# mims-harvard/ProCyon

Measured on AMD Instinct MI355X. Metric: phenotype-gen tokens/sec (ProCyon-Full greedy generation, end to end), higher is better.
Workload: dtype bf16; 1 GPU; configs[1]: ProCyon-Full (ESM2-650M + Llama-3-8B geometry=full) bf16 batch=1, 1024-residue protein, 512-token prompt, 256-token greedy generation; parallelism=single GPU

## Files before the change

### procyon_amd/_lib.py

```python
from __future__ import annotations

import ctypes as C
import os

_HERE = os.path.dirname(os.path.abspath(__file__))
LIB_PATH = os.environ.get("PCY_LIB") or os.path.join(_HERE, "libpcy.so")

EPI_STORE, EPI_RESID, EPI_GELU_ERF, EPI_GELU_ESM, EPI_SWIGLU = range(5)
POOL_MEAN, POOL_MEAN_CORRECTED, POOL_MAX = range(3)
ABI_VERSION = 10
(DISPATCH_GEMM_128, DISPATCH_GEMM_64, DISPATCH_GEMM_BIG, DISPATCH_GEMM_BIG_PERSIST, DISPATCH_GEMM_SPLITK, DISPATCH_GEMM_FP8, DISPATCH_ATTN_FAST,
 DISPATCH_DEC_STEP_GQA, DISPATCH_GEMM_MID, DISPATCH_ESM_GRAPH, DISPATCH_DEC_STEP_MHA, DISPATCH_DEC_LAYER, DISPATCH_DEC_STEP_NB, DISPATCH_DEC_STEP_MB,
 DISPATCH_DEC_LOOP_STREAM, DISPATCH_DEC_LOOP_MFMA) = range(16)
DISPATCH_DECODE = dict(step_gqa=DISPATCH_DEC_STEP_GQA, step_mha=DISPATCH_DEC_STEP_MHA, layer=DISPATCH_DEC_LAYER, step_nb=DISPATCH_DEC_STEP_NB,
                       step_mb=DISPATCH_DEC_STEP_MB, loop_stream=DISPATCH_DEC_LOOP_STREAM, loop_mfma=DISPATCH_DEC_LOOP_MFMA)

vp = C.c_void_p
i32 = C.c_int32
ci = C.c_int


class MlpDesc(C.Structure):
    _fields_ = [("n_layers", i32), ("dims", i32 * 9), ("w", vp * 8), ("b", vp * 8)]


class EsmLayer(C.Structure):
    _fields_ = [(n, vp) for n in ("wqkv", "bqkv", "wo", "bo", "ln1_w", "ln1_b", "w1", "b1", "w2", "b2", "ln2_w", "ln2_b")]


class EsmDesc(C.Structure):
    _fields_ = [("d", i32), ("n_layers", i32), ("n_heads", i32), ("ffn", i32), ("vocab", i32), ("ln_eps", C.c_float),
                ("rope_mode", i32), ("embed", vp), ("final_ln_w", vp), ("final_ln_b", vp), ("rope_cos", vp),
                ("rope_sin", vp), ("layers", C.POINTER(EsmLayer))]


class LlamaLayer(C.Structure):
# ... 118 lines not shown
```

### procyon_amd/csrc/pcy_elem.hip

```cpp
#include "pcy_internal.h"

namespace {

constexpr int NT = 256;

__global__ __launch_bounds__(NT) void rmsnorm_kernel(const bf16_t* __restrict__ x, const bf16_t* __restrict__ w,
                                                     bf16_t* __restrict__ y, int d, float eps, int cast) {
  __shared__ float red[NT / 64];
  const bf16_t* xr = x + (size_t)blockIdx.x * d;
  bf16_t* yr = y + (size_t)blockIdx.x * d;
  float ss = 0.f;
  for (int k = threadIdx.x * 8; k < d; k += NT * 8) {
    const uint4 v = *reinterpret_cast<const uint4*>(xr + k);
    const uint32_t u[4] = {v.x, v.y, v.z, v.w};
#pragma unroll
    for (int j = 0; j < 4; ++j) { float a = lo_bf(u[j]), b = hi_bf(u[j]); ss += a * a + b * b; }
  }
  ss = block_sum<NT>(ss, red);
  const float rstd = rsqrtf(ss / (float)d + eps);
  for (int k = threadIdx.x * 8; k < d; k += NT * 8) {
    const uint4 v = *reinterpret_cast<const uint4*>(xr + k);
    const uint4 g = *reinterpret_cast<const uint4*>(w + k);
    const uint32_t u[4] = {v.x, v.y, v.z, v.w}, gg[4] = {g.x, g.y, g.z, g.w};
    uint32_t o[4];
// ... 334 lines not shown
      wsum[((size_t)p * POOL_CH + ch) * d + c + e] = a;
      wcnt[((size_t)p * POOL_CH + ch) * d + c + e] = n;
    }
  }
}
__global__ __launch_bounds__(NT) void pool_finish_kernel(const float* __restrict__ wsum, const int* __restrict__ wcnt, int d, int mode,
                                                         bf16_t* __restrict__ out) {
  const int p = blockIdx.x, c = blockIdx.y * NT + threadIdx.x;
  if (c >= d) return;
  float a = wsum[(size_t)p * POOL_CH * d + c];
  int n = wcnt[(size_t)p * POOL_CH * d + c];
  for (int ch = 1; ch < POOL_CH; ++ch) {
    const float v = wsum[((size_t)p * POOL_CH + ch) * d + c];
    if (mode == 2) a = fmaxf(a, v);
    else { a += v; n += wcnt[((size_t)p * POOL_CH + ch) * d + c]; }
  }
  out[(size_t)p * d + c] = (mode == 2) ? f2bf(a) : f2bf(rbf(a) / (float)n);
}

constexpr int PICK_NT = 256;
constexpr int PICK_NB = 64;
struct PickPartial { float mx; int idx; float se; int pad; };

__global__ __launch_bounds__(PICK_NT) void pick_stage1_kernel(const bf16_t* __restrict__ logits, int V, PickPartial* __restrict__ part) {
  __shared__ float redv[PICK_NT / 64];
  __shared__ int redi[PICK_NT / 64];
  __shared__ float red[PICK_NT / 64];
  const int b = blockIdx.y, c = blockIdx.x;
  const int chunk = (V + PICK_NB - 1) / PICK_NB;
  const int lo = c * chunk, hi = (lo + chunk) < V ? (lo + chunk) : V;
  const bf16_t* lg = logits + (size_t)b * V;
  float best = -INFINITY;
  int bi = 0x7fffffff;
  for (int i = lo + threadIdx.x; i < hi; i += PICK_NT) {
    const float v = bf2f(lg[i]);
    if (v > best || (v == best && i < bi)) { best = v; bi = i; }
  }
#pragma unroll
  for (int o = 32; o > 0; o >>= 1) {
    const float ov = __shfl_xor(best, o, 64);
    const int oi = __shfl_xor(bi, o, 64);
    if (ov > best || (ov == best && oi < bi)) { best = ov; bi = oi; }
  }
  const int w = threadIdx.x >> 6;
  if ((threadIdx.x & 63) == 0) { redv[w] = best; redi[w] = bi; }
  __syncthreads();
  best = redv[0]; bi = redi[0];
  for (int i = 1; i < PICK_NT / 64; ++i)
    if (redv[i] > best || (redv[i] == best && redi[i] < bi)) { best = redv[i]; bi = redi[i]; }
  float se = 0.f;
  for (int i = lo + threadIdx.x; i < hi; i += PICK_NT) se += expf(bf2f(lg[i]) - best);
  se = block_sum<PICK_NT>(se, red);
  if (threadIdx.x == 0) part[b * PICK_NB + c] = PickPartial{best, bi, (lo < hi) ? se : 0.f, 0};
}

__global__ __launch_bounds__(256) void pick_stage2_kernel(const bf16_t* __restrict__ logits, int V, const PickPartial* __restrict__ part,
                                                          int32_t* __restrict__ next_tok, int32_t* __restrict__ tokens_out, int max_steps,
                                                          float* __restrict__ logprob, int32_t* __restrict__ step_dev, int32_t* __restrict__ pos_dev,
                                                          int advance_pos, int B) {
  const int l = threadIdx.x & 63;
  const int step = *step_dev;
  for (int b = threadIdx.x >> 6; b < B; b += 4) {
    const PickPartial pp = part[b * PICK_NB + l];
    float best = pp.mx;
    int bi = pp.idx;
#pragma unroll
    for (int o = 32; o > 0; o >>= 1) {
      const float ov = __shfl_xor(best, o, 64);
      const int oi = __shfl_xor(bi, o, 64);
      if (ov > best || (ov == best && oi < bi)) { best = ov; bi = oi; }
    }
    float se = pp.se * expf(pp.mx - best);
    se = wave_sum(se);
    if (l == 0) {
      const float lsm = rbf((bf2f(logits[(size_t)b * V + bi]) - best) - logf(se));
      logprob[b] += lsm;
      next_tok[b] = bi;
      tokens_out[(size_t)b * max_steps + step] = bi;
    }
  }
  __syncthreads();
  if (threadIdx.x == 0) { if (advance_pos) *pos_dev += 1; *step_dev = step + 1; }
}

constexpr int SMP_NT = 1024;

__global__ __launch_bounds__(PICK_NT) void sample_stage1_kernel(const bf16_t* __restrict__ logits, int V, float temperature,
                                                                float4* __restrict__ part) {
  __shared__ float red[PICK_NT / 64];
  const int b = blockIdx.y, c = blockIdx.x;
  const int chunk = (V + PICK_NB - 1) / PICK_NB;
  const int lo = c * chunk, hi = (lo + chunk) < V ? (lo + chunk) : V;
  const bf16_t* lg = logits + (size_t)b * V;
  const bool scaled = temperature != 1.0f;
  float mr = -INFINITY, ms = -INFINITY;
  for (int i = lo + threadIdx.x; i < hi; i += PICK_NT) {
    const float v = bf2f(lg[i]);
    mr = fmaxf(mr, v);
    ms = fmaxf(ms, scaled ? rbf(v / temperature) : v);
  }
  mr = block_max<PICK_NT>(mr, red);
  ms = block_max<PICK_NT>(ms, red);
  float sr = 0.f, ss = 0.f;
  for (int i = lo + threadIdx.x; i < hi; i += PICK_NT) {
    const float v = bf2f(lg[i]);
// ... 832 lines not shown
    for (int q = 0; q < nseq; ++q) { out[q] = acc; acc += (cu[q + 1] - cu[q] + pad - 1) / pad * pad; }
    out[nseq] = acc;
  }
}
void pcy_launch_vt_offsets(hipStream_t s, const int32_t* cu, int nseq, int pad, int32_t* vt_cu_out) {
  hipLaunchKernelGGL(vt_offsets_kernel, dim3(1), dim3(64), 0, s, cu, nseq, pad, vt_cu_out);
}
void pcy_launch_transpose_v(hipStream_t s, const bf16_t* buf, int ld, int vcol0, int nh, int dh, const int32_t* cu,
                            const int32_t* vt_cu, int nseq, int max_len, bf16_t* vt, int vt_total) {
  if (nseq <= 0) return;
  const int maxpad = (max_len + 63) / 64 * 64;
  hipLaunchKernelGGL(transpose_v_kernel, dim3((maxpad + 63) / 64, nh * dh / 64, nseq), dim3(NT), 0, s, buf, ld, vcol0, dh, cu, vt_cu, vt, vt_total);
}
size_t pcy_pool_ws_bytes(int nprot, int d) { return (size_t)nprot * POOL_CH * d * 8; }
void pcy_launch_pool(hipStream_t s, const bf16_t* h, int d, const int32_t* seg, const int32_t* rng, int nprot, int mode, bf16_t* out,
                     void* ws) {
  if (nprot <= 0) return;
  float* wsum = reinterpret_cast<float*>(ws);
  int* wcnt = reinterpret_cast<int*>(wsum + (size_t)nprot * POOL_CH * d);
  hipLaunchKernelGGL(pool_partial_kernel, dim3(nprot, (d + 511) / 512, POOL_CH), dim3(NT), 0, s, h, d, seg, rng, mode, wsum, wcnt);
  hipLaunchKernelGGL(pool_finish_kernel, dim3(nprot, (d + NT - 1) / NT), dim3(NT), 0, s, wsum, wcnt, d, mode, out);
}
void pcy_launch_greedy_pick(hipStream_t s, const bf16_t* logits, int B, int V, int32_t* next_tok, int32_t* tokens_out,
                            int max_steps, float* logprob, int32_t* pos_dev, int32_t* step_dev, int advance_pos, void* partials) {
  hipLaunchKernelGGL(pick_stage1_kernel, dim3(PICK_NB, B), dim3(PICK_NT), 0, s, logits, V, reinterpret_cast<PickPartial*>(partials));
  hipLaunchKernelGGL(pick_stage2_kernel, dim3(1), dim3(256), 0, s, logits, V, reinterpret_cast<const PickPartial*>(partials), next_tok,
                     tokens_out, max_steps, logprob, step_dev, pos_dev, advance_pos, B);
}
int pcy_sample_max_vocab() { return SMP_NT * SMP_KMAX; }
void pcy_launch_sample_step(hipStream_t s, const bf16_t* logits, int B, int V, float temperature, float nucleus_p, const float* uniforms,
                            unsigned* hist, bf16_t* probs_out, int32_t* next_tok, int32_t* tokens_out, int max_steps, float* logprob,
                            int32_t* pos_dev, int32_t* step_dev, int advance_pos, void* partials, bf16_t* pbits) {
  hipLaunchKernelGGL(sample_stage1_kernel, dim3(PICK_NB, B), dim3(PICK_NT), 0, s, logits, V, temperature, reinterpret_cast<float4*>(partials));
  hipLaunchKernelGGL(sample_probs_kernel, dim3(PICK_NB, B), dim3(PICK_NT), 0, s, logits, V, reinterpret_cast<const float4*>(partials), temperature,
                     nucleus_p > 0.f ? 1 : 0, hist, pbits);
  hipLaunchKernelGGL(sample_stage2_kernel, dim3(B), dim3(SMP_NT), 0, s, logits, V, reinterpret_cast<const float4*>(partials), temperature,
                     nucleus_p, uniforms, hist, probs_out, next_tok, tokens_out, max_steps, logprob, step_dev, B, pbits);
  hipLaunchKernelGGL(sample_advance_kernel, dim3(1), dim3(64), 0, s, pos_dev, step_dev, advance_pos);
}
void pcy_launch_copy_rows(hipStream_t s, const bf16_t* src, int lds_, bf16_t* dst, int ldd, const int32_t* rows, int nrows, int d) {
  if (nrows > 0) hipLaunchKernelGGL(copy_rows_kernel, dim3(nrows), dim3(NT), 0, s, src, lds_, dst, ldd, rows, d);
}
void pcy_launch_l2norm_rows(hipStream_t s, const bf16_t* x, bf16_t* y, int rows, int d, float eps) {
  if (rows > 0) hipLaunchKernelGGL(l2norm_rows_kernel, dim3(rows), dim3(NT), 0, s, x, y, d, eps);
}
void pcy_launch_retrieval_rank(hipStream_t s, const bf16_t* sims, int Q, int N, int k, int32_t* idx_out, bf16_t* score_out) {
  if (Q > 0 && N > 0 && k > 0)
// ... 34 lines not shown
```

### procyon_amd/csrc/pcy_engine.hip

```cpp
#include <stdio.h>
#include <stdlib.h>
#include <stdarg.h>
#include <string.h>
#include <dlfcn.h>
#include <vector>

#include "../../include/pcy.h"
#include "pcy_internal.h"

namespace {

thread_local char g_err[512] = "";

int fail(int code, const char* fmt, ...) {
  va_list ap;
  va_start(ap, fmt);
  vsnprintf(g_err, sizeof(g_err), fmt, ap);
  va_end(ap);
  return code;
}

#define HIP_TRY(expr)                                                                       \
  do {                                                                                      \
    hipError_t e_ = (expr);                                                                 \
// ... 1 lines not shown
  } while (0)

inline size_t align_up(size_t v, size_t a) { return (v + a - 1) / a * a; }

}

void pcy_set_error(const char* fmt, ...) {
  va_list ap;
  va_start(ap, fmt);
  vsnprintf(g_err, sizeof(g_err), fmt, ap);
  va_end(ap);
}

struct DecodeGraphKey {
  int kind;
  int B;
  PcySwitches sw;
  const void *model, *layers, *embed, *kv_k, *kv_v, *pos, *step, *next_tok, *logits, *keep;
  int Tmax, kv_B;
  const void *ws, *mc_tags, *mb_flags, *nb_tags, *dev_layers;
  uint64_t layers_fp;
  const void *tokens_out, *logprob, *logits_all;
  int logits_all_ld, max_steps;
  pcy_beam_state beam_state;
  const void *logits_rec, *beam_ws;
  int beam, group_size, kv_t0;
  uint32_t penalty_bits;
};

struct pcy_ctx {
  int device = 0;
  hipStream_t stream = nullptr;
  hipStream_t cap_stream = nullptr;
  char* ws = nullptr;
  size_t ws_bytes = 0;
  hipEvent_t ev0 = nullptr, ev1 = nullptr;
  hipGraphExec_t graph = nullptr;
  DecodeGraphKey graph_key = {};
  int n_cu = 0;
  unsigned* xwg_err = nullptr;
  unsigned* ao_sync = nullptr;
  uint32_t* mc_tags = nullptr;
  const void* mc_tags_model = nullptr;
  size_t mc_tags_words = 0;
  PcySwitches mc_tags_sw = {};
  uint64_t layers_fp = 0;
  PcyLayerWeightsDev* dev_layers = nullptr;
  uint32_t* nb_tags[9] = {};
  unsigned* nb_sync = nullptr;
  unsigned* mb_flags = nullptr;
  size_t mb_flags_words = 0;
  unsigned* mb_sync = nullptr;
  uint32_t* op_tags = nullptr;
  size_t op_tags_words = 0;
  unsigned* smp_hist = nullptr;
  int smp_hist_rows = 0;
  bf16_t* smp_pbits = nullptr;
  size_t smp_pbits_elems = 0;
  char* beam_ws = nullptr;
  size_t beam_ws_bytes = 0;

  struct GraphSlot { uint64_t key[16]; hipGraphExec_t exec; unsigned long long stamp; };
  static constexpr int N_GSLOTS = 8;
  GraphSlot gslots[N_GSLOTS] = {};
  unsigned long long gstamp = 0;
  void drop_gslots() {
    for (auto& g : gslots) {
      if (g.exec) hipGraphExecDestroy(g.exec);
      g = GraphSlot{};
    }
  }

  int reserve(size_t bytes) {
    static const bool poison = [] { const char* e = getenv("PCY_DEBUG_POISON_WS"); return e && atoi(e) != 0; }();
    if (poison && ws && bytes <= ws_bytes) HIP_TRY(hipMemsetAsync(ws, 0xFF, ws_bytes, stream));
    if (bytes <= ws_bytes) return 0;
    if (ws) {
      HIP_TRY(hipStreamSynchronize(stream));
      HIP_TRY(hipFree(ws));
      ws = nullptr; ws_bytes = 0;
    }
    drop_graph();
// ... 66 lines not shown
}
bool decode_mb_covers(const pcy_ctx* c, const pcy_llama_desc* m, int B, const PcySwitches& sw) {
  return B >= 9 && B <= 32 && B <= sw.mb_max && m->d == 4096 && m->ffn == 14336 && m->n_heads == 32 && m->n_kv_heads == 8 && m->head_dim == 128 && c->n_cu >= 256;
}
size_t tag_words_per_layer(const pcy_llama_desc* m) {
  return (size_t)m->ffn + (size_t)m->d + (size_t)(m->n_heads + 2 * m->n_kv_heads) * m->head_dim + (size_t)m->n_heads * m->head_dim;
}

int ensure_sync_words(pcy_ctx* c) {
  if (!c->n_cu) {
    hipDeviceProp_t prop;
    HIP_TRY(hipGetDeviceProperties(&prop, c->device));
    c->n_cu = prop.multiProcessorCount;
  }
  if (!c->xwg_err) {
    HIP_TRY(hipHostMalloc(reinterpret_cast<void**>(&c->xwg_err), 64, hipHostMallocMapped | hipHostMallocCoherent));
    memset(c->xwg_err, 0, 64);
  }
  if (!c->ao_sync) {
    const size_t bytes = (size_t)(64 + 2 * AO_MAX_LAYERS * AO_FLAGS) * sizeof(unsigned);
    HIP_TRY(hipMalloc(reinterpret_cast<void**>(&c->ao_sync), bytes));
    HIP_TRY(hipMemset(c->ao_sync, 0, bytes));
  }
  return 0;
}
uint64_t layers_fingerprint(const pcy_llama_desc* m) {
  uint64_t h = 1469598103934665603ull;
  auto mix = [&](const void* p) { h = (h ^ (uint64_t)(uintptr_t)p) * 1099511628211ull; };
  mix(m->layers);
  for (int l = 0; l < m->n_layers; ++l) {
    const pcy_llama_layer& L = m->layers[l];
    mix(L.ln1); mix(L.wqkv); mix(L.wo); mix(L.ln2); mix(L.wgu); mix(L.wdown);
  }
  return h;
}
int ensure_decode_state(pcy_ctx* c, const pcy_llama_desc* m, int B, const PcySwitches& sw) {
  if (int r = ensure_sync_words(c)) return r;
  const size_t words = (size_t)m->n_layers * (tag_words_per_layer(m) + 32 * 256);
  const uint64_t fp = layers_fingerprint(m);
  if (c->mc_tags_model != m || c->mc_tags_words != words || c->mc_tags_sw != sw || c->layers_fp != fp) {
    HIP_TRY(hipStreamSynchronize(c->stream));
    c->drop_graph();
    if (c->mc_tags) HIP_TRY(hipFree(c->mc_tags));
    c->mc_tags = nullptr;
    HIP_TRY(hipMalloc(reinterpret_cast<void**>(&c->mc_tags), words * 4));
    HIP_TRY(hipMemset(c->mc_tags, 0, words * 4));
// ... 156 lines not shown
  PcyDecodeStepArgs sa{};
  sa.layers = cx.c->dev_layers; sa.n_layers = cx.m->n_layers; sa.kv_layer_stride = cx.layer_stride;
  sa.tags = tags; sa.tag_stride = tag_stride; sa.xflags_stride = xflags_stride;
  sa.x_lines = tags + (size_t)cx.m->n_layers * tag_stride; sa.x_lines_stride = line_stride;
  return sa;
}
PcyGemvArgs proj_args(const DecodeCx& cx, const DecodePlan& p, const void* W, const void* ln, const bf16_t* in, int K, bf16_t* out, int N, int epi,
                      bool splitk, int krot, int* xn_ready) {
  const pcy_llama_desc* m = cx.m;
  PcyGemvArgs g{};
  g.W = (const bf16_t*)W; g.x = in; g.y = out; g.N = N; g.K = K; g.B = cx.B; g.ldx = K; g.ldy = N; g.epi = epi;
  g.force_stream = p.nb_on; g.krot = krot;
  if (splitk) { g.splitk_ws = cx.sk_ws; g.splitk_ws_bytes = cx.sk_bytes; }
  if (epi == EPI_RESID) {
    g.resid = out;
    if (p.batched && cx.B <= 32) { g.next_rms_w = (const bf16_t*)ln; g.next_xn = cx.xn; g.fused_next = xn_ready; g.rms_eps = m->rms_eps; g.rms_cast = m->rms_cast; }
  } else {
    g.rms_eps = m->rms_eps; g.rms_cast = m->rms_cast;
    if (p.batched) g.x = cx.xn; else g.rms_w = (const bf16_t*)ln;
  }
  return g;
}

void enqueue_decode(pcy_ctx* c, const pcy_llama_desc* m, const pcy_kv_cache* kv, const pcy_gen_state* st, int B, const PcySwitches& sw, bool layers_only = false) {
  hipStream_t s = c->stream;
  const int d = m->d, H = m->n_heads, dh = m->head_dim, F = m->ffn;
  const DecodeCx cx = decode_cx(c, m, kv, st, B);
  const DecodePlan p = plan_decode(c, m, kv, B, sw);
  if (layers_only) {
    if (p.epoch_word) pcy_launch_bump(s, p.epoch_word);
    if (p.tag_word) pcy_launch_bump(s, p.tag_word);
  } else {
    pcy_launch_embed_tokens_dev(s, (const bf16_t*)m->embed, st->next_tok, cx.x, B, d, p.epoch_word, p.tag_word);
  }
  const size_t tag_stride = tag_words_per_layer(m);
  bool step_done = false;
  bool try_layer = p.path == DEC_STEP_GQA || p.path == DEC_STEP_MHA || p.path == DEC_LAYERS;
  int xn_ready = 0;
  if (p.path == DEC_STEP_NB) {
    const PcyDecodeStepArgs sa = step_args(cx, c->nb_tags[B], pcy_decode_nb_tag_words(B), 2 * AO_FLAGS, pcy_decode_nb_line_words(B));
    step_done = pcy_launch_decode_step_nb(s, c->device, attn_args(cx, p, -1), block_args(cx, p.tag_word, mc_trace(sw)), mlp_args(cx, p.tag_word), sa, c->n_cu,
                                          c->ao_sync, B, sw.nb_ub);
    if (step_done) ++g_pcy_dispatch[PCY_DISPATCH_DEC_STEP_NB];
  } else if (p.path == DEC_STEP_GQA || p.path == DEC_STEP_MHA) {
    const PcyDecodeStepArgs sa = step_args(cx, c->mc_tags, tag_stride, AO_FLAGS, 32 * 256);
    step_done = pcy_launch_decode_step(s, attn_args(cx, p, -1), block_args(cx, p.tag_word, mc_trace(sw)), mlp_args(cx, p.tag_word), sa, c->n_cu,
                                       c->ao_sync);
  } else if (p.path == DEC_STEP_MB) {
    PcyMbArgs ma{};
    ma.layers = c->dev_layers; ma.n_layers = m->n_layers; ma.final_norm = (const bf16_t*)m->final_norm;
    ma.x = cx.x; ma.xn = cx.xn; ma.ao = cx.ao; ma.act = cx.act;
    ma.qkv_ws = cx.sk_ws; ma.sk_ws = cx.sk_ws + (size_t)2 * B * cx.qkvw;
    ma.kcache = (bf16_t*)kv->k; ma.vcache = (bf16_t*)kv->v; ma.kv_layer_stride = cx.layer_stride; ma.Bcache = kv->B;
    ma.pos_dev = st->pos; ma.cos_t = (const bf16_t*)m->rope_cos; ma.sin_t = (const bf16_t*)m->rope_sin; ma.keep = st->keep; ma.ld_keep = kv->Tmax;
    ma.B = B; ma.Tmax = kv->Tmax; ma.scale = 1.0f / sqrtf((float)dh); ma.rms_eps = m->rms_eps; ma.rms_cast = m->rms_cast;
// ... 48 lines not shown
}

__global__ void store_logits_kernel(const bf16_t* __restrict__ logits, bf16_t* __restrict__ all, const int32_t* step_dev,
                                    int B, int V, int ld) {
  const size_t step = (size_t)(*step_dev);
  const int chunks = (V + 7) / 8;
  const bool vec = (ld % 8 == 0) && ((reinterpret_cast<uintptr_t>(all) & 15) == 0);
  for (size_t i = (size_t)blockIdx.x * blockDim.x + threadIdx.x; i < (size_t)B * chunks; i += (size_t)gridDim.x * blockDim.x) {
    const int b = (int)(i / chunks), c = (int)(i % chunks);
    const bf16_t* src = logits + (size_t)b * V + c * 8;
    bf16_t* dst = all + (step * B + b) * ld + c * 8;
    if (vec && c * 8 + 8 <= V) {
      const uint32_t w0 = src[0] | ((uint32_t)src[1] << 16), w1 = src[2] | ((uint32_t)src[3] << 16);
      const uint32_t w2 = src[4] | ((uint32_t)src[5] << 16), w3 = src[6] | ((uint32_t)src[7] << 16);
      *reinterpret_cast<uint4*>(dst) = make_uint4(w0, w1, w2, w3);
    } else {
      for (int e = 0; e < 8 && c * 8 + e < V; ++e) dst[e] = src[e];
    }
  }
}
void enqueue_store_logits(hipStream_t s, const void* logits, void* all, int ld, const int32_t* step_dev, int B, int V) {
  if (all) hipLaunchKernelGGL(store_logits_kernel, dim3(B >= 8 ? 256 : 64), dim3(256), 0, s, (const bf16_t*)logits, (bf16_t*)all, step_dev, B, V, ld > 0 ? ld : V);
}
void enqueue_pick(pcy_ctx* c, const pcy_llama_desc* m, const pcy_gen_state* st, int B, int advance_pos, int Tmax) {
  enqueue_store_logits(c->stream, st->logits, st->logits_all, st->logits_all_ld, st->step, B, m->vocab);
  pcy_launch_greedy_pick(c->stream, (const bf16_t*)st->logits, B, m->vocab, st->next_tok, st->tokens_out, st->max_steps,
                         st->logprob, st->pos, st->step, advance_pos, carve_decode_ws(c->ws, m, B, Tmax).partials);
}

void enqueue_sample(pcy_ctx* c, const pcy_llama_desc* m, const pcy_gen_state* st, int B, int advance_pos, int Tmax, float temperature,
                    float nucleus_p, const float* uniforms, bf16_t* probs_out) {
  hipStream_t s = c->stream;
  if (nucleus_p > 0.f) temperature = 1.0f;
  enqueue_store_logits(s, st->logits, st->logits_all, st->logits_all_ld, st->step, B, m->vocab);
  void* partials = carve_decode_ws(c->ws, m, B, Tmax).partials;
  pcy_launch_sample_step(s, (const bf16_t*)st->logits, B, m->vocab, temperature, nucleus_p, uniforms, c->smp_hist, probs_out, st->next_tok,
                         st->tokens_out, st->max_steps, st->logprob, st->pos, st->step, advance_pos, partials, c->smp_pbits);
}
int ensure_sample_state(pcy_ctx* c, int B, int V) {
  if ((size_t)B * V > c->smp_pbits_elems) {
    if (c->smp_pbits) { HIP_TRY(hipStreamSynchronize(c->stream)); HIP_TRY(hipFree(c->smp_pbits)); c->smp_pbits = nullptr; c->smp_pbits_elems = 0; }
    HIP_TRY(hipMalloc(reinterpret_cast<void**>(&c->smp_pbits), (size_t)B * V * 2));
    c->smp_pbits_elems = (size_t)B * V;
  }
  if (B <= c->smp_hist_rows) return 0;
  if (c->smp_hist) { HIP_TRY(hipStreamSynchronize(c->stream)); HIP_TRY(hipFree(c->smp_hist)); c->smp_hist = nullptr; }
  HIP_TRY(hipMalloc(reinterpret_cast<void**>(&c->smp_hist), (size_t)B * 65536 * sizeof(unsigned)));
  HIP_TRY(hipMemset(c->smp_hist, 0, (size_t)B * 65536 * sizeof(unsigned)));
  c->smp_hist_rows = B;
  return 0;
// ... 83 lines not shown
  c->stream = reinterpret_cast<hipStream_t>(stream);
  HIP_TRY(hipEventCreate(&c->ev0));
  HIP_TRY(hipEventCreate(&c->ev1));
  HIP_TRY(hipStreamCreateWithFlags(&c->cap_stream, hipStreamNonBlocking));
  *out = c;
  return 0;
}
void pcy_ctx_destroy(pcy_ctx* c) {
  if (!c) return;
  hipStreamSynchronize(c->stream);
  c->drop_graph();
  c->drop_gslots();
  if (c->ws) hipFree(c->ws);
  if (c->xwg_err) hipHostFree(c->xwg_err);
  if (c->ao_sync) hipFree(c->ao_sync);
  if (c->mc_tags) hipFree(c->mc_tags);
  if (c->dev_layers) hipFree(c->dev_layers);
  for (auto& t : c->nb_tags) if (t) hipFree(t);
  if (c->nb_sync) hipFree(c->nb_sync);
  if (c->mb_flags) hipFree(c->mb_flags);
  if (c->mb_sync) hipFree(c->mb_sync);
  if (c->op_tags) hipFree(c->op_tags);
  if (c->beam_ws) hipFree(c->beam_ws);
  if (c->smp_hist) hipFree(c->smp_hist);
  if (c->smp_pbits) hipFree(c->smp_pbits);
  if (c->ev0) hipEventDestroy(c->ev0);
  if (c->ev1) hipEventDestroy(c->ev1);
  if (c->cap_stream) hipStreamDestroy(c->cap_stream);
  delete c;
}
int pcy_ctx_sync(pcy_ctx* c) {
  HIP_TRY(hipStreamSynchronize(c->stream));
  return take_sticky_error(c);
}
int pcy_timer_start(pcy_ctx* c) { HIP_TRY(hipEventRecord(c->ev0, c->stream)); return 0; }
int pcy_timer_stop(pcy_ctx* c, float* ms) {
  HIP_TRY(hipEventRecord(c->ev1, c->stream));
  HIP_TRY(hipEventSynchronize(c->ev1));
  HIP_TRY(hipEventElapsedTime(ms, c->ev0, c->ev1));
  return 0;
}

int pcy_gemm(pcy_ctx* c, const void* A, int lda, const void* W, const void* bias, const void* resid, int ldr, void* C,
             int ldc, int M, int N, int K, int epi) {
  if (K % 64 != 0) return fail(1, "pcy_gemm: K=%d must be a multiple of 64", K);
  if (epi == EPI_SWIGLU && N % 32 != 0) return fail(1, "pcy_gemm: SwiGLU needs N %% 32 == 0");
// ... 592 lines not shown
  if (!c->graph || memcmp(&key, &c->graph_key, sizeof(key)) != 0) {
    c->drop_graph();
    hipGraph_t g = nullptr;
    hipStream_t user = c->stream;
    c->stream = c->cap_stream;
    hipError_t e0 = hipStreamBeginCapture(c->cap_stream, hipStreamCaptureModeThreadLocal);
    if (e0 == hipSuccess) {
      enqueue();
      e0 = hipStreamEndCapture(c->cap_stream, &g);
    }
    c->stream = user;
    if (e0 != hipSuccess) return fail(2, "%s graph capture failed: %s", what, hipGetErrorString(e0));
    HIP_TRY(hipGraphInstantiate(&c->graph, g, nullptr, nullptr, 0));
    hipGraphDestroy(g);
    memcpy(&c->graph_key, &key, sizeof(key));
  }
  for (int i = 0; i < n_steps; ++i) HIP_TRY(hipGraphLaunch(c->graph, c->stream));
  return 0;
}
int replay_decode_graph(pcy_ctx* c, const pcy_llama_desc* m, const pcy_kv_cache* kv, const pcy_gen_state* st, int B, int n_steps, int kind, const PcySwitches& sw) {
  DecodeGraphKey key;
  decode_graph_key(key, c, m, kv, st, B, kind, sw);
  key.tokens_out = st->tokens_out; key.logprob = st->logprob; key.logits_all = st->logits_all; key.logits_all_ld = st->logits_all_ld; key.max_steps = st->max_steps;
  return replay_graph(c, key, n_steps, "decode-step", [&] {
    enqueue_decode(c, m, kv, st, B, sw);
    if (kind == 0) enqueue_pick(c, m, st, B, 1, kv->Tmax);
  });
}
}
extern "C" {
int pcy_llama_prefill(pcy_ctx* c, const pcy_llama_desc* m, const pcy_kv_cache* kv, const void* embeds, const uint8_t* keep,
                      const int32_t* pos, const int32_t* cu, const int32_t* vt_cu, int B, int T, const int32_t* logit_rows,
                      int n_logit_rows, void* logits_out, void* hidden_out, const int32_t* sum_rows, int n_sum_rows,
                      void* hidden_sum_out) {
  return llama_prefill_impl(c, m, kv, embeds, keep, pos, cu, vt_cu, B, T, logit_rows, n_logit_rows, logits_out, hidden_out, sum_rows,
                            n_sum_rows, hidden_sum_out, nullptr);
}
int pcy_llama_prefill_all(pcy_ctx* c, const pcy_llama_desc* m, const pcy_kv_cache* kv, const void* embeds, const uint8_t* keep,
                          const int32_t* pos, const int32_t* cu, const int32_t* vt_cu, int B, int T, const int32_t* logit_rows,
                          int n_logit_rows, void* logits_out, void* hidden_all_out) {
  if (!hidden_all_out) return fail(1, "pcy_llama_prefill_all: hidden_all_out is NULL");
  return llama_prefill_impl(c, m, kv, embeds, keep, pos, cu, vt_cu, B, T, logit_rows, n_logit_rows, logits_out, nullptr, nullptr, 0,
                            nullptr, hidden_all_out);
}

int pcy_llama_decode(pcy_ctx* c, const pcy_llama_desc* m, const pcy_kv_cache* kv, const pcy_gen_state* st, int B) {
  PCY_STICKY(c);
  if (B > kv->B) return fail(1, "pcy_llama_decode: B=%d exceeds cache rows %d", B, kv->B);
  if (int r = c->reserve(decode_ws_bytes(m, B, kv->Tmax))) return r;
  const PcySwitches sw = pcy_read_switches();
  if (int r = ensure_decode_state(c, m, B, sw)) return r;
  enqueue_decode(c, m, kv, st, B, sw);
  return check_launch("pcy_llama_decode");
}

int pcy_llama_decode_layers(pcy_ctx* c, const pcy_llama_desc* m, const pcy_kv_cache* kv, const pcy_gen_state* st, int B, int reps) {
  PCY_STICKY(c);
  if (B > kv->B) return fail(1, "pcy_llama_decode_layers: B=%d exceeds cache rows %d", B, kv->B);
  if (int r = c->reserve(decode_ws_bytes(m, B, kv->Tmax))) return r;
  const PcySwitches sw = pcy_read_switches();
  if (int r = ensure_decode_state(c, m, B, sw)) return r;
  for (int i = 0; i < reps; ++i) enqueue_decode(c, m, kv, st, B, sw, true);
  return check_launch("pcy_llama_decode_layers");
}

int pcy_greedy_pick(pcy_ctx* c, const pcy_llama_desc* m, const pcy_kv_cache* kv, const pcy_gen_state* st, int B, int advance_pos) {
  PCY_STICKY(c);
  if (int r = c->reserve(decode_ws_bytes(m, B, kv->Tmax))) return r;
  enqueue_pick(c, m, st, B, advance_pos, kv->Tmax);
  return check_launch("pcy_greedy_pick");
}


int pcy_llama_greedy(pcy_ctx* c, const pcy_llama_desc* m, const pcy_kv_cache* kv, const pcy_gen_state* st, int B, int n_steps,
                     int use_graph) {
  PCY_STICKY(c);
  if (B > kv->B) return fail(1, "pcy_llama_greedy: B=%d exceeds cache rows %d", B, kv->B);
  if (int r = c->reserve(decode_ws_bytes(m, B, kv->Tmax))) return r;
  const PcySwitches sw = pcy_read_switches();
  if (int r = ensure_decode_state(c, m, B, sw)) return r;
  if (!use_graph) {
    for (int i = 0; i < n_steps; ++i) {
      enqueue_decode(c, m, kv, st, B, sw);
      enqueue_pick(c, m, st, B, 1, kv->Tmax);
    }
    return check_launch("pcy_llama_greedy");
  }
  return replay_decode_graph(c, m, kv, st, B, n_steps, 0, sw);
}

int pcy_llama_decode_graph(pcy_ctx* c, const pcy_llama_desc* m, const pcy_kv_cache* kv, const pcy_gen_state* st, int B) {
  PCY_STICKY(c);
  if (B > kv->B) return fail(1, "pcy_llama_decode_graph: B=%d exceeds cache rows %d", B, kv->B);
  if (int r = c->reserve(decode_ws_bytes(m, B, kv->Tmax))) return r;
  const PcySwitches sw = pcy_read_switches();
  if (int r = ensure_decode_state(c, m, B, sw)) return r;
  return replay_decode_graph(c, m, kv, st, B, 1, 1, sw);
}

int pcy_sample_pick(pcy_ctx* c, const pcy_llama_desc* m, const pcy_kv_cache* kv, const pcy_gen_state* st, int B, int advance_pos,
                    float temperature, float nucleus_prob, const float* uniforms, void* probs_out) {
  PCY_STICKY(c);
  if (!(temperature > 0.f)) return fail(1, "pcy_sample_pick: temperature must be > 0 (greedy: pcy_greedy_pick)");
  if (nucleus_prob >= 1.f) return fail(1, "pcy_sample_pick: nucleus_prob must be < 1 (<= 0 switches the nucleus mask off)");
  if (m->vocab > pcy_sample_max_vocab()) return fail(1, "pcy_sample_pick: vocabulary %d unsupported (<= %d)", m->vocab, pcy_sample_max_vocab());
  if (int r = c->reserve(decode_ws_bytes(m, B, kv->Tmax))) return r;
  if (int r = ensure_sample_state(c, B, m->vocab)) return r;
// ... 100 lines not shown
```

### procyon_amd/csrc/pcy_internal.h

```cpp
#pragma once
#include "pcy_common.h"
#include "pcy_switch.h"

struct PcyGemvArgs {
  const bf16_t* W;
  const bf16_t* x;
  bf16_t* y;
  const bf16_t* bias;
  const bf16_t* resid;
  const bf16_t* rms_w;
  float rms_eps;
  int rms_cast;
  int N, K, B, ldx, ldy, epi;
  int plain_loads;
  float* splitk_ws; size_t splitk_ws_bytes;
  const bf16_t* next_rms_w; bf16_t* next_xn; int* fused_next;
  int* defer_finish;
  int force_stream;
  int force_mfma;
  int krot;
};
void pcy_launch_gemv(hipStream_t s, const PcyGemvArgs& a);

__host__ __device__ inline int pcy_gemv_kshift(int r0_wg, int nss) {
// ... 38 lines not shown
  int gn;
  const int32_t* rope_pos; const bf16_t* rope_cos; const bf16_t* rope_sin; int rope_ncols, rope_qcols, rope_mode; float rope_scale;
  float* splitk_ws; size_t splitk_ws_bytes;
  int fp8; const float* sa; const float* sw;
  const bf16_t* next_rms_w; bf16_t* next_xn; int* fused_next; float rms_eps; int rms_cast;
  int gelu_select;
  int mid_cfg;
};
struct pcy_ctx;
hipStream_t pcy_ctx_stream(pcy_ctx* c);
void pcy_set_error(const char* fmt, ...);
void pcy_launch_gemm(hipStream_t s, const PcyGemmArgs& a);
void pcy_gemm_prepare(hipStream_t s);
enum { PCY_DISPATCH_GEMM_128 = 0, PCY_DISPATCH_GEMM_64 = 1, PCY_DISPATCH_GEMM_BIG = 2, PCY_DISPATCH_GEMM_BIG_PERSIST = 3,
       PCY_DISPATCH_GEMM_SPLITK = 4, PCY_DISPATCH_GEMM_FP8 = 5, PCY_DISPATCH_ATTN_FAST = 6,
       PCY_DISPATCH_DEC_STEP_GQA = 7,
       PCY_DISPATCH_GEMM_MID = 8, PCY_DISPATCH_ESM_GRAPH = 9,
       PCY_DISPATCH_DEC_STEP_MHA = 10,
       PCY_DISPATCH_DEC_LAYER = 11,
       PCY_DISPATCH_DEC_STEP_NB = 12,
       PCY_DISPATCH_DEC_STEP_MB = 13,
       PCY_DISPATCH_DEC_LOOP_STREAM = 14,
       PCY_DISPATCH_DEC_LOOP_MFMA = 15,
       PCY_DISPATCH_N = 16 };
extern unsigned long long g_pcy_dispatch[PCY_DISPATCH_N];

void pcy_launch_quant_rows_fp8(hipStream_t s, const bf16_t* x, int ldx, int rows, int K, unsigned char* q, float* scale);
bool pcy_launch_rmsnorm_quant_fp8(hipStream_t s, const bf16_t* x, const bf16_t* w, int rows, int d, float eps, int cast,
                                  unsigned char* q, float* scale);
void pcy_launch_rmsnorm(hipStream_t s, const bf16_t* x, const bf16_t* w, bf16_t* y, int rows, int d, float eps, int cast);
void pcy_launch_layernorm(hipStream_t s, const bf16_t* x, const bf16_t* w, const bf16_t* b, bf16_t* y, int rows, int d, float eps);
void pcy_launch_embed_gather(hipStream_t s, const bf16_t* table, const int32_t* ids, const bf16_t* soft,
                             const int32_t* soft_map, bf16_t* out, int rows, int d);
void pcy_launch_embed_tokens_dev(hipStream_t s, const bf16_t* table, const int32_t* ids, bf16_t* out, int rows, int d, unsigned* epoch = nullptr,
                                 unsigned* epoch2 = nullptr);
void pcy_launch_esm_embed(hipStream_t s, const bf16_t* table, const int32_t* toks, const int32_t* cu, int nseq,
                          int max_len, bf16_t* out, int d, int mask_pads);
void pcy_launch_rope(hipStream_t s, bf16_t* buf, int ld, int col0, int nh, int dh, const int32_t* pos,
                     const bf16_t* cos_t, const bf16_t* sin_t, int ntok, int mode, float prescale);
bool pcy_launch_prefill_post_qkv(hipStream_t s, bf16_t* qkv, int ld, int H, int Hkv, int dh, const int32_t* pos, const bf16_t* cos_t,
                                 const bf16_t* sin_t, bf16_t* kcache, bf16_t* vcache, int B, int T, int Tmax, const int32_t* cu,
                                 const int32_t* vt_cu, bf16_t* vt, int vt_total);
void pcy_launch_kv_scatter(hipStream_t s, const bf16_t* qkv, int ld, int kcol0, int vcol0, int Hkv, int dh,
                           bf16_t* kcache, bf16_t* vcache, int B, int T, int Tmax);
void pcy_launch_transpose_v(hipStream_t s, const bf16_t* buf, int ld, int vcol0, int nh, int dh, const int32_t* cu,
                            const int32_t* vt_cu, int nseq, int max_len, bf16_t* vt, int vt_total);

// ... 76 lines not shown
  bf16_t* x;
  bf16_t* xn;
  bf16_t* ao;
  bf16_t* act;
  float* qkv_ws;
  float* sk_ws;
  bf16_t* kcache; bf16_t* vcache; size_t kv_layer_stride; int Bcache;
  const int32_t* pos_dev; const bf16_t* cos_t; const bf16_t* sin_t; const uint8_t* keep; int ld_keep;
  int B, Tmax; float scale, rms_eps; int rms_cast;
  unsigned* flags;
  const unsigned* epoch;
  unsigned* err;
  unsigned long long* trace;
  int abl;
};
size_t pcy_decode_mb_flag_words();
int pcy_decode_mb_ds(int B);
bool pcy_decode_mb_fits(int B, int Tmax);
bool pcy_launch_decode_step_mb(hipStream_t s, int device, const PcyMbArgs& a, int n_cu);

size_t pcy_pool_ws_bytes(int nprot, int d);
void pcy_launch_pool(hipStream_t s, const bf16_t* h, int d, const int32_t* seg, const int32_t* rng, int nprot,
                     int mode, bf16_t* out, void* ws);
void pcy_launch_greedy_pick(hipStream_t s, const bf16_t* logits, int B, int V, int32_t* next_tok, int32_t* tokens_out,
                            int max_steps, float* logprob, int32_t* pos_dev, int32_t* step_dev, int advance_pos,
                            void* partials );
void pcy_launch_retrieval_dot_f32(hipStream_t s, const float* query, int Q, const void* targets, int targets_bf16, int N, int D, float eps, float* sims);
size_t pcy_retrieval_dot_smem(int D);
void pcy_launch_retrieval_rank_f32(hipStream_t s, const float* sims, int Q, int N, int k, int32_t* idx_out, float* score_out);
int pcy_sample_max_vocab();
void pcy_launch_sample_step(hipStream_t s, const bf16_t* logits, int B, int V, float temperature, float nucleus_p, const float* uniforms,
                            unsigned* hist, bf16_t* probs_out, int32_t* next_tok, int32_t* tokens_out, int max_steps, float* logprob,
                            int32_t* pos_dev, int32_t* step_dev, int advance_pos, void* partials ,
                            bf16_t* pbits );
struct PcyBeamState {
  int32_t* out; int32_t max_len;
  float* cur; float* cur_new;
  int32_t* next_tok;
  int32_t* src;
  int32_t* anc;
  uint8_t* has_eos;
  int32_t* blk_eos; int32_t* ticket;
  int32_t* pos; int32_t* step; int32_t* done;
  int32_t eos_id;
};
size_t pcy_beam_ws_bytes(int B, int beam);
void pcy_launch_beam_step(hipStream_t s, const bf16_t* logits, int V, int B, int beam, int g, float penalty, const PcyBeamState& st,
                          void* ws);
void pcy_launch_copy_rows(hipStream_t s, const bf16_t* src, int lds, bf16_t* dst, int ldd, const int32_t* rows,
// ... 6 lines not shown
```

### procyon_amd/csrc/pcy_switch.h

```cpp
#pragma once
#include <stdint.h>
#include <stdlib.h>
#include <string.h>
#include <type_traits>

#define PCY_SWITCH_NAMES(X)                                                                                                                \
  X(attn_o) X(mlp_chain) X(decode_layer) X(decode_step) X(attn_qkv_finish) X(finish_norm) X(fp8_fused_norm) X(prefill_post_qkv) X(gemv_lds) \
  X(gemv_mfma4) X(fa_vrow) X(gelu_fast) X(esm_graph) X(lds_prefetch) X(decode_nb) X(decode_nb_step) X(beam_graph) X(kv_permute)             \
  X(decode_mb_step) X(beam_prefill_once) X(beam_kv_suffix)
enum PcySwitch {
#define X(n) PCY_SW_##n,
  PCY_SWITCH_NAMES(X)
#undef X
  PCY_SW_COUNT
};
static_assert(PCY_SW_COUNT <= 32, "PcySwitches::off_mask holds one bit per name");

inline bool pcy_list_has(const char* list, const char* name) {
  if (!list) return false;
  const size_t n = strlen(name);
  for (const char* p = list; (p = strstr(p, name)) != nullptr; p += n)
    if ((p == list || p[-1] == ',') && (p[n] == 0 || p[n] == ',')) return true;
  return false;
}
inline bool pcy_off(const char* name) { return pcy_list_has(getenv("PCY_DISABLE"), name); }

struct PcySwitches {
  uint32_t off_mask;
  int32_t nb_max, mb_max;
  int32_t xmin[3];
  int32_t nb_ub;
  int32_t mb_abl;
// ... 31 lines not shown
```

Measured before the change: 395.1 tokens/s.

## Fuse greedy pick, logits record and next-token embed into one tail kernel

Replaces the per-step store-logits, pick stage1, pick stage2 and next-token embedding launches with a single token_tail kernel. It uses a last-block-done atomic ticket to merge partials and then writes the next token's embedding row and bumps the epoch/tag words, so the following decode step skips its own embed launch. This is meant to remove several small kernel launches and their serialization on the per-token critical path. The cost is more complex cross-block synchronization through a global ticket with release/acquire fences, and a prologue embed launch before the loop.

```diff
diff --git a/procyon_amd/_lib.py b/procyon_amd/_lib.py
--- a/procyon_amd/_lib.py
+++ b/procyon_amd/_lib.py
@@ -11,7 +11,7 @@
 ABI_VERSION = 10
 (DISPATCH_GEMM_128, DISPATCH_GEMM_64, DISPATCH_GEMM_BIG, DISPATCH_GEMM_BIG_PERSIST, DISPATCH_GEMM_SPLITK, DISPATCH_GEMM_FP8, DISPATCH_ATTN_FAST,
  DISPATCH_DEC_STEP_GQA, DISPATCH_GEMM_MID, DISPATCH_ESM_GRAPH, DISPATCH_DEC_STEP_MHA, DISPATCH_DEC_LAYER, DISPATCH_DEC_STEP_NB, DISPATCH_DEC_STEP_MB,
- DISPATCH_DEC_LOOP_STREAM, DISPATCH_DEC_LOOP_MFMA) = range(16)
+ DISPATCH_DEC_LOOP_STREAM, DISPATCH_DEC_LOOP_MFMA, DISPATCH_TOKEN_TAIL) = range(17)
 DISPATCH_DECODE = dict(step_gqa=DISPATCH_DEC_STEP_GQA, step_mha=DISPATCH_DEC_STEP_MHA, layer=DISPATCH_DEC_LAYER, step_nb=DISPATCH_DEC_STEP_NB,
                        step_mb=DISPATCH_DEC_STEP_MB, loop_stream=DISPATCH_DEC_LOOP_STREAM, loop_mfma=DISPATCH_DEC_LOOP_MFMA)
 
diff --git a/procyon_amd/csrc/pcy_elem.hip b/procyon_amd/csrc/pcy_elem.hip
--- a/procyon_amd/csrc/pcy_elem.hip
+++ b/procyon_amd/csrc/pcy_elem.hip
@@ -380,11 +380,9 @@
 constexpr int PICK_NB = 64;
 struct PickPartial { float mx; int idx; float se; int pad; };
 
-__global__ __launch_bounds__(PICK_NT) void pick_stage1_kernel(const bf16_t* __restrict__ logits, int V, PickPartial* __restrict__ part) {
-  __shared__ float redv[PICK_NT / 64];
-  __shared__ int redi[PICK_NT / 64];
-  __shared__ float red[PICK_NT / 64];
-  const int b = blockIdx.y, c = blockIdx.x;
+struct PickLds { float redv[PICK_NT / 64]; int redi[PICK_NT / 64]; float red[PICK_NT / 64]; };
+
+__device__ __forceinline__ void pick_scan_chunk(const bf16_t* __restrict__ logits, int V, PickPartial* __restrict__ part, int b, int c, PickLds& sm) {
   const int chunk = (V + PICK_NB - 1) / PICK_NB;
   const int lo = c * chunk, hi = (lo + chunk) < V ? (lo + chunk) : V;
   const bf16_t* lg = logits + (size_t)b * V;
@@ -401,44 +399,113 @@
     if (ov > best || (ov == best && oi < bi)) { best = ov; bi = oi; }
   }
   const int w = threadIdx.x >> 6;
-  if ((threadIdx.x & 63) == 0) { redv[w] = best; redi[w] = bi; }
-  __syncthreads();
-  best = redv[0]; bi = redi[0];
+  if ((threadIdx.x & 63) == 0) { sm.redv[w] = best; sm.redi[w] = bi; }
+  __syncthreads();
+  best = sm.redv[0]; bi = sm.redi[0];
   for (int i = 1; i < PICK_NT / 64; ++i)
-    if (redv[i] > best || (redv[i] == best && redi[i] < bi)) { best = redv[i]; bi = redi[i]; }
+    if (sm.redv[i] > best || (sm.redv[i] == best && sm.redi[i] < bi)) { best = sm.redv[i]; bi = sm.redi[i]; }
   float se = 0.f;
   for (int i = lo + threadIdx.x; i < hi; i += PICK_NT) se += expf(bf2f(lg[i]) - best);
-  se = block_sum<PICK_NT>(se, red);
+  se = block_sum<PICK_NT>(se, sm.red);
   if (threadIdx.x == 0) part[b * PICK_NB + c] = PickPartial{best, bi, (lo < hi) ? se : 0.f, 0};
+}
+
+__device__ __forceinline__ int pick_merge_row(const bf16_t* __restrict__ logits, int V, const PickPartial* __restrict__ part, int b, int step,
+                                              int32_t* __restrict__ next_tok, int32_t* __restrict__ tokens_out, int max_steps,
+                                              float* __restrict__ logprob) {
+  const int l = threadIdx.x & 63;
+  const PickPartial pp = part[b * PICK_NB + l];
+  float best = pp.mx;
+  int bi = pp.idx;
+#pragma unroll
+  for (int o = 32; o > 0; o >>= 1) {
+    const float ov = __shfl_xor(best, o, 64);
+    const int oi = __shfl_xor(bi, o, 64);
+    if (ov > best || (ov == best && oi < bi)) { best = ov; bi = oi; }
+  }
+  float se = pp.se * expf(pp.mx - best);
+  se = wave_sum(se);
+  if (l == 0) {
+    const float lsm = rbf((bf2f(logits[(size_t)b * V + bi]) - best) - logf(se));
+    logprob[b] += lsm;
+    next_tok[b] = bi;
+    tokens_out[(size_t)b * max_steps + step] = bi;
+  }
+  return bi;
+}
+
+__global__ __launch_bounds__(PICK_NT) void pick_stage1_kernel(const bf16_t* __restrict__ logits, int V, PickPartial* __restrict__ part) {
+  __shared__ PickLds sm;
+  pick_scan_chunk(logits, V, part, blockIdx.y, blockIdx.x, sm);
 }
 
 __global__ __launch_bounds__(256) void pick_stage2_kernel(const bf16_t* __restrict__ logits, int V, const PickPartial* __restrict__ part,
                                                           int32_t* __restrict__ next_tok, int32_t* __restrict__ tokens_out, int max_steps,
                                                           float* __restrict__ logprob, int32_t* __restrict__ step_dev, int32_t* __restrict__ pos_dev,
                                                           int advance_pos, int B) {
+  const int step = *step_dev;
+  for (int b = threadIdx.x >> 6; b < B; b += 4) pick_merge_row(logits, V, part, b, step, next_tok, tokens_out, max_steps, logprob);
+  __syncthreads();
+  if (threadIdx.x == 0) { if (advance_pos) *pos_dev += 1; *step_dev = step + 1; }
+}
+
+__global__ __launch_bounds__(PICK_NT) void token_tail_kernel(const bf16_t* __restrict__ logits, int V, PickPartial* __restrict__ part,
+                                                             int32_t* __restrict__ next_tok, int32_t* __restrict__ tokens_out, int max_steps,
+                                                             float* __restrict__ logprob, int32_t* __restrict__ step_dev, int32_t* __restrict__ pos_dev,
+                                                             int advance_pos, PcyTokenTail t) {
+  __shared__ PickLds sm;
+  const int b = blockIdx.y, c = blockIdx.x, B = gridDim.y;
+  const int step = *step_dev;
+  if (t.record) {
+    const int units = (V + 7) / 8;
+    const bool vec = (t.record_ld % 8 == 0) && ((reinterpret_cast<uintptr_t>(t.record) & 15) == 0);
+    const bf16_t* srow = logits + (size_t)b * V;
+    bf16_t* drow = t.record + ((size_t)step * B + b) * t.record_ld;
+    for (int u = c * PICK_NT + threadIdx.x; u < units; u += PICK_NB * PICK_NT) {
+      const bf16_t* src = srow + u * 8;
+      bf16_t* dst = drow + u * 8;
+      if (vec && u * 8 + 8 <= V) {
+        const uint32_t w0 = src[0] | ((uint32_t)src[1] << 16), w1 = src[2] | ((uint32_t)src[3] << 16);
+        const uint32_t w2 = src[4] | ((uint32_t)src[5] << 16), w3 = src[6] | ((uint32_t)src[7] << 16);
+        *reinterpret_cast<uint4*>(dst) = make_uint4(w0, w1, w2, w3);
+      } else {
+        for (int e = 0; e < 8 && u * 8 + e < V; ++e) dst[e] = src[e];
+      }
+    }
+  }
+  pick_scan_chunk(logits, V, part, b, c, sm);
+  asm volatile("s_waitcnt vmcnt(0)" ::: "memory");
+  __syncthreads();
+  if (threadIdx.x == 0) {
+    __builtin_amdgcn_fence(__ATOMIC_RELEASE, "agent");
+    asm volatile("s_waitcnt vmcnt(0)" ::: "memory");
+    const unsigned ticket = __hip_atomic_fetch_add(t.ticket, 1u, __ATOMIC_RELAXED, __HIP_MEMORY_SCOPE_AGENT);
+    sm.redi[0] = ticket == (unsigned)(PICK_NB * B) - 1u;
+  }
+  __syncthreads();
+  if (!sm.redi[0]) return;
+  __builtin_amdgcn_fence(__ATOMIC_ACQUIRE, "agent");
+  asm volatile("s_waitcnt vmcnt(0)" ::: "memory");
+  __syncthreads();
   const int l = threadIdx.x & 63;
-  const int step = *step_dev;
-  for (int b = threadIdx.x >> 6; b < B; b += 4) {
-    const PickPartial pp = part[b * PICK_NB + l];
-    float best = pp.mx;
-    int bi = pp.idx;
-#pragma unroll
-    for (int o = 32; o > 0; o >>= 1) {
-      const float ov = __shfl_xor(best, o, 64);
-      const int oi = __shfl_xor(bi, o, 64);
-      if (ov > best || (ov == best && oi < bi)) { best = ov; bi = oi; }
-    }
-    float se = pp.se * expf(pp.mx - best);
-    se = wave_sum(se);
-    if (l == 0) {
-      const float lsm = rbf((bf2f(logits[(size_t)b * V + bi]) - best) - logf(se));
-      logprob[b] += lsm;
-      next_tok[b] = bi;
-      tokens_out[(size_t)b * max_steps + step] = bi;
-    }
-  }
-  __syncthreads();
-  if (threadIdx.x == 0) { if (advance_pos) *pos_dev += 1; *step_dev = step + 1; }
+  for (int r = threadIdx.x >> 6; r < B; r += PICK_NT / 64) {
+    const int tok = pick_merge_row(logits, V, part, r, step, next_tok, tokens_out, max_steps, logprob);
+    if (t.embed && (unsigned)tok < (unsigned)V) {
+      const bf16_t* src = t.embed + (size_t)tok * t.d;
+      bf16_t* dst = t.x + (size_t)r * t.d;
+      for (int k = l * 8; k < t.d; k += 64 * 8) *reinterpret_cast<uint4*>(dst + k) = *reinterpret_cast<const uint4*>(src + k);
+    }
+  }
+  __syncthreads();
+  if (threadIdx.x == 0) {
+    __hip_atomic_store(t.ticket, 0u, __ATOMIC_RELAXED, __HIP_MEMORY_SCOPE_AGENT);
+    if (t.embed) {
+      if (t.epoch) *t.epoch += 1;
+      if (t.epoch2) *t.epoch2 += 1;
+    }
+    if (advance_pos) *pos_dev += 1;
+    *step_dev = step + 1;
+  }
 }
 
 constexpr int SMP_NT = 1024;
@@ -1317,7 +1384,12 @@
   hipLaunchKernelGGL(pool_finish_kernel, dim3(nprot, (d + NT - 1) / NT), dim3(NT), 0, s, wsum, wcnt, d, mode, out);
 }
 void pcy_launch_greedy_pick(hipStream_t s, const bf16_t* logits, int B, int V, int32_t* next_tok, int32_t* tokens_out,
-                            int max_steps, float* logprob, int32_t* pos_dev, int32_t* step_dev, int advance_pos, void* partials) {
+                            int max_steps, float* logprob, int32_t* pos_dev, int32_t* step_dev, int advance_pos, void* partials, const PcyTokenTail* tail) {
+  if (tail) {
+    hipLaunchKernelGGL(token_tail_kernel, dim3(PICK_NB, B), dim3(PICK_NT), 0, s, logits, V, reinterpret_cast<PickPartial*>(partials), next_tok,
+                       tokens_out, max_steps, logprob, step_dev, pos_dev, advance_pos, *tail);
+    return;
+  }
   hipLaunchKernelGGL(pick_stage1_kernel, dim3(PICK_NB, B), dim3(PICK_NT), 0, s, logits, V, reinterpret_cast<PickPartial*>(partials));
   hipLaunchKernelGGL(pick_stage2_kernel, dim3(1), dim3(256), 0, s, logits, V, reinterpret_cast<const PickPartial*>(partials), next_tok,
                      tokens_out, max_steps, logprob, step_dev, pos_dev, advance_pos, B);
diff --git a/procyon_amd/csrc/pcy_engine.hip b/procyon_amd/csrc/pcy_engine.hip
--- a/procyon_amd/csrc/pcy_engine.hip
+++ b/procyon_amd/csrc/pcy_engine.hip
@@ -47,6 +47,7 @@
   uint64_t layers_fp;
   const void *tokens_out, *logprob, *logits_all;
   int logits_all_ld, max_steps;
+  const void *tail_ticket, *tail_x;
   pcy_beam_state beam_state;
   const void *logits_rec, *beam_ws;
   int beam, group_size, kv_t0;
@@ -83,6 +84,7 @@
   bf16_t* smp_pbits = nullptr;
   size_t smp_pbits_elems = 0;
   char* beam_ws = nullptr;
+  unsigned* tail_ticket = nullptr;
   size_t beam_ws_bytes = 0;
 
   struct GraphSlot { uint64_t key[16]; hipGraphExec_t exec; unsigned long long stamp; };
@@ -195,6 +197,13 @@
     HIP_TRY(hipMalloc(reinterpret_cast<void**>(&c->ao_sync), bytes));
     HIP_TRY(hipMemset(c->ao_sync, 0, bytes));
   }
+  return 0;
+}
+int ensure_tail_ticket(pcy_ctx* c) {
+  if (c->tail_ticket) return 0;
+  HIP_TRY(hipMalloc(reinterpret_cast<void**>(&c->tail_ticket), 64));
+  HIP_TRY(hipMemset(c->tail_ticket, 0, 64));
+  HIP_TRY(hipDeviceSynchronize());
   return 0;
 }
 uint64_t layers_fingerprint(const pcy_llama_desc* m) {
@@ -397,7 +406,12 @@
   return g;
 }
 
-void enqueue_decode(pcy_ctx* c, const pcy_llama_desc* m, const pcy_kv_cache* kv, const pcy_gen_state* st, int B, const PcySwitches& sw, bool layers_only = false) {
+void enqueue_embed(pcy_ctx* c, const pcy_llama_desc* m, const pcy_kv_cache* kv, const pcy_gen_state* st, int B, const PcySwitches& sw) {
+  const DecodePlan p = plan_decode(c, m, kv, B, sw);
+  pcy_launch_embed_tokens_dev(c->stream, (const bf16_t*)m->embed, st->next_tok, carve_decode_ws(c->ws, m, B, kv->Tmax).x, B, m->d, p.epoch_word, p.tag_word);
+}
+void enqueue_decode(pcy_ctx* c, const pcy_llama_desc* m, const pcy_kv_cache* kv, const pcy_gen_state* st, int B, const PcySwitches& sw, bool layers_only = false,
+                    bool embedded = false) {
   hipStream_t s = c->stream;
   const int d = m->d, H = m->n_heads, dh = m->head_dim, F = m->ffn;
   const DecodeCx cx = decode_cx(c, m, kv, st, B);
@@ -405,7 +419,7 @@
   if (layers_only) {
     if (p.epoch_word) pcy_launch_bump(s, p.epoch_word);
     if (p.tag_word) pcy_launch_bump(s, p.tag_word);
-  } else {
+  } else if (!embedded) {
     pcy_launch_embed_tokens_dev(s, (const bf16_t*)m->embed, st->next_tok, cx.x, B, d, p.epoch_word, p.tag_word);
   }
   const size_t tag_stride = tag_words_per_layer(m);
@@ -500,10 +514,24 @@
 void enqueue_store_logits(hipStream_t s, const void* logits, void* all, int ld, const int32_t* step_dev, int B, int V) {
   if (all) hipLaunchKernelGGL(store_logits_kernel, dim3(B >= 8 ? 256 : 64), dim3(256), 0, s, (const bf16_t*)logits, (bf16_t*)all, step_dev, B, V, ld > 0 ? ld : V);
 }
-void enqueue_pick(pcy_ctx* c, const pcy_llama_desc* m, const pcy_gen_state* st, int B, int advance_pos, int Tmax) {
-  enqueue_store_logits(c->stream, st->logits, st->logits_all, st->logits_all_ld, st->step, B, m->vocab);
+void enqueue_pick(pcy_ctx* c, const pcy_llama_desc* m, const pcy_gen_state* st, int B, int advance_pos, int Tmax, const PcySwitches& sw,
+                  const pcy_kv_cache* embed_next = nullptr) {
+  const DecodeWs ws = carve_decode_ws(c->ws, m, B, Tmax);
+  if (sw.off(PCY_SW_token_tail)) {
+    enqueue_store_logits(c->stream, st->logits, st->logits_all, st->logits_all_ld, st->step, B, m->vocab);
+    pcy_launch_greedy_pick(c->stream, (const bf16_t*)st->logits, B, m->vocab, st->next_tok, st->tokens_out, st->max_steps,
+                           st->logprob, st->pos, st->step, advance_pos, ws.partials);
+    return;
+  }
+  PcyTokenTail t{};
+  t.record = (bf16_t*)st->logits_all; t.record_ld = st->logits_all_ld > 0 ? st->logits_all_ld : m->vocab; t.ticket = c->tail_ticket;
+  if (embed_next) {
+    const DecodePlan p = plan_decode(c, m, embed_next, B, sw);
+    t.embed = (const bf16_t*)m->embed; t.x = ws.x; t.d = m->d; t.epoch = p.epoch_word; t.epoch2 = p.tag_word;
+  }
   pcy_launch_greedy_pick(c->stream, (const bf16_t*)st->logits, B, m->vocab, st->next_tok, st->tokens_out, st->max_steps,
-                         st->logprob, st->pos, st->step, advance_pos, carve_decode_ws(c->ws, m, B, Tmax).partials);
+                         st->logprob, st->pos, st->step, advance_pos, ws.partials, &t);
+  ++g_pcy_dispatch[PCY_DISPATCH_TOKEN_TAIL];
 }
 
 void enqueue_sample(pcy_ctx* c, const pcy_llama_desc* m, const pcy_gen_state* st, int B, int advance_pos, int Tmax, float temperature,
@@ -633,6 +661,7 @@
   if (c->mb_sync) hipFree(c->mb_sync);
   if (c->op_tags) hipFree(c->op_tags);
   if (c->beam_ws) hipFree(c->beam_ws);
+  if (c->tail_ticket) hipFree(c->tail_ticket);
   if (c->smp_hist) hipFree(c->smp_hist);
   if (c->smp_pbits) hipFree(c->smp_pbits);
   if (c->ev0) hipEventDestroy(c->ev0);
@@ -1271,9 +1300,11 @@
   DecodeGraphKey key;
   decode_graph_key(key, c, m, kv, st, B, kind, sw);
   key.tokens_out = st->tokens_out; key.logprob = st->logprob; key.logits_all = st->logits_all; key.logits_all_ld = st->logits_all_ld; key.max_steps = st->max_steps;
+  const bool tail = kind == 0 && !sw.off(PCY_SW_token_tail);
+  if (tail) { key.tail_ticket = c->tail_ticket; key.tail_x = carve_decode_ws(c->ws, m, B, kv->Tmax).x; }
   return replay_graph(c, key, n_steps, "decode-step", [&] {
-    enqueue_decode(c, m, kv, st, B, sw);
-    if (kind == 0) enqueue_pick(c, m, st, B, 1, kv->Tmax);
+    enqueue_decode(c, m, kv, st, B, sw, false, tail);
+    if (kind == 0) enqueue_pick(c, m, st, B, 1, kv->Tmax, sw, tail ? kv : nullptr);
   });
 }
 }
@@ -1316,7 +1347,10 @@
 int pcy_greedy_pick(pcy_ctx* c, const pcy_llama_desc* m, const pcy_kv_cache* kv, const pcy_gen_state* st, int B, int advance_pos) {
   PCY_STICKY(c);
   if (int r = c->reserve(decode_ws_bytes(m, B, kv->Tmax))) return r;
-  enqueue_pick(c, m, st, B, advance_pos, kv->Tmax);
+  const PcySwitches sw = pcy_read_switches();
+  if (!sw.off(PCY_SW_token_tail))
+    if (int r = ensure_tail_ticket(c)) return r;
+  enqueue_pick(c, m, st, B, advance_pos, kv->Tmax, sw);
   return check_launch("pcy_greedy_pick");
 }
 
@@ -1328,10 +1362,15 @@
   if (int r = c->reserve(decode_ws_bytes(m, B, kv->Tmax))) return r;
   const PcySwitches sw = pcy_read_switches();
   if (int r = ensure_decode_state(c, m, B, sw)) return r;
+  const bool tail = !sw.off(PCY_SW_token_tail);
+  if (tail && n_steps > 0) {
+    if (int r = ensure_tail_ticket(c)) return r;
+    enqueue_embed(c, m, kv, st, B, sw);
+  }
   if (!use_graph) {
     for (int i = 0; i < n_steps; ++i) {
-      enqueue_decode(c, m, kv, st, B, sw);
-      enqueue_pick(c, m, st, B, 1, kv->Tmax);
+      enqueue_decode(c, m, kv, st, B, sw, false, tail);
+      enqueue_pick(c, m, st, B, 1, kv->Tmax, sw, tail ? kv : nullptr);
     }
     return check_launch("pcy_llama_greedy");
   }
diff --git a/procyon_amd/csrc/pcy_internal.h b/procyon_amd/csrc/pcy_internal.h
--- a/procyon_amd/csrc/pcy_internal.h
+++ b/procyon_amd/csrc/pcy_internal.h
@@ -84,7 +84,8 @@
        PCY_DISPATCH_DEC_STEP_MB = 13,
        PCY_DISPATCH_DEC_LOOP_STREAM = 14,
        PCY_DISPATCH_DEC_LOOP_MFMA = 15,
-       PCY_DISPATCH_N = 16 };
+       PCY_DISPATCH_TOKEN_TAIL = 16,
+       PCY_DISPATCH_N = 17 };
 extern unsigned long long g_pcy_dispatch[PCY_DISPATCH_N];
 
 void pcy_launch_quant_rows_fp8(hipStream_t s, const bf16_t* x, int ldx, int rows, int K, unsigned char* q, float* scale);
@@ -207,9 +208,15 @@
 size_t pcy_pool_ws_bytes(int nprot, int d);
 void pcy_launch_pool(hipStream_t s, const bf16_t* h, int d, const int32_t* seg, const int32_t* rng, int nprot,
                      int mode, bf16_t* out, void* ws);
+struct PcyTokenTail {
+  bf16_t* record; int record_ld;
+  const bf16_t* embed; bf16_t* x; int d;
+  unsigned* epoch; unsigned* epoch2;
+  unsigned* ticket;
+};
 void pcy_launch_greedy_pick(hipStream_t s, const bf16_t* logits, int B, int V, int32_t* next_tok, int32_t* tokens_out,
                             int max_steps, float* logprob, int32_t* pos_dev, int32_t* step_dev, int advance_pos,
-                            void* partials );
+                            void* partials , const PcyTokenTail* tail = nullptr);
 void pcy_launch_retrieval_dot_f32(hipStream_t s, const float* query, int Q, const void* targets, int targets_bf16, int N, int D, float eps, float* sims);
 size_t pcy_retrieval_dot_smem(int D);
 void pcy_launch_retrieval_rank_f32(hipStream_t s, const float* sims, int Q, int N, int k, int32_t* idx_out, float* score_out);
diff --git a/procyon_amd/csrc/pcy_switch.h b/procyon_amd/csrc/pcy_switch.h
--- a/procyon_amd/csrc/pcy_switch.h
+++ b/procyon_amd/csrc/pcy_switch.h
@@ -7,7 +7,7 @@
 #define PCY_SWITCH_NAMES(X)                                                                                                                \
   X(attn_o) X(mlp_chain) X(decode_layer) X(decode_step) X(attn_qkv_finish) X(finish_norm) X(fp8_fused_norm) X(prefill_post_qkv) X(gemv_lds) \
   X(gemv_mfma4) X(fa_vrow) X(gelu_fast) X(esm_graph) X(lds_prefetch) X(decode_nb) X(decode_nb_step) X(beam_graph) X(kv_permute)             \
-  X(decode_mb_step) X(beam_prefill_once) X(beam_kv_suffix)
+  X(decode_mb_step) X(beam_prefill_once) X(beam_kv_suffix) X(token_tail)
 enum PcySwitch {
 #define X(n) PCY_SW_##n,
   PCY_SWITCH_NAMES(X)
```

Result: no change. 395.8 tokens/s, median of 6 (+0.2%).
